# massquantity/dismember

Hardware: AMD Instinct MI355X
Metric: beam-search users/sec + recall@200 vs brute-force, 10M-item tree (higher is better)
Workload: dtype f32; 1 GPU; TDM beam-search serving, synthetic 10000000-item depth-24 binary tree, 128-d emb, beam=200, topk=200, L=10; items=10000000, depth=24, embed=128, beam=200, topk=200, seq_len=10, parallelism=user-sharded x1, replicated table

## Files before the change

dismember_amd/csrc/beam_kernel.hip.inc:

```

#if !defined(DM_PROBE_BUILD) &&                                                                                            \
    (defined(DM_DBG_NO_S) || defined(DM_DBG_NO_GATHER) || defined(DM_DBG_NO_EPI) || defined(DM_DBG_NO_XLANE) ||             \
     defined(DM_SPLIT_NO_MIX) || defined(DMW_DBG_F_NOEPI) || defined(DMW_DBG_F_NOLD) || defined(DMW_DBG_F_NOSM) ||          \
     defined(DMW_DBG_HOTROWS) || defined(DMW_DBG_NOWAIT) || defined(DMW_DBG_NO_GATHER) || defined(DMW_DBG_NO_GVV) ||        \
     defined(DMW_DBG_SM_UPTO) || defined(DM_PHASE_TIMERS) || defined(DM_TILE_TIMERS) || defined(DM_SETUP_TIMERS))
#error "timing knock-outs and in-kernel timers need -DDM_PROBE_BUILD (probe builds only: they change results)"
#endif

typedef float f32x4 __attribute__((ext_vector_type(4)));
typedef _Float16 dm_h8 __attribute__((ext_vector_type(8)));
typedef _Float16 dm_h2 __attribute__((ext_vector_type(2)));

#define DM_BLOCK 512
#define DM_NWAVES 8
#define DM_MAXL 16
#define DM_PIPE_MAXL 32

struct BeamParams {
  const float *emb;
  const f32x4 *wfrag;
  const f32x4 *afrag;
  const f32x4 *bfrag;
  const float *b1, *w2;
  float b2;
  const dm_h8 *wsplit;
  const dm_h8 *emb_split;
  float emb_scale, score_unscale, acc_scale, out_unscale;
  int64_t num_index;
  const uint32_t *exists_bits, *leaf_bits;
  const int32_t *node_id, *id_to_code;
  int64_t n_slots;
  int32_t non_leaf_offset, max_code, max_level;
  int leaf_fast;
  const int32_t *seq;
  int64_t U;
  int L, use_mask, beam, topk, widen;
  const int64_t *consumed_off;
  const int32_t *consumed_ids;
  int mode;
  const int32_t *bf_leaf_codes;
  int64_t bf_n_leaf;
  int bf_slices, bf_chunk;
  int64_t bf_per_slice;
  unsigned long long *bf_out_keys;
  int otm_leaf_level;
  int nteams, cap, pcap;
  int32_t *out_ids;
  float *out_scores;
  int32_t *out_counts;
  int out_stride;
  int32_t *ws_code;
  float *ws_score;
  uint32_t *ws_khi, *ws_klo;
  int ws_cap;
  unsigned long long *next_user;
  int32_t *trace_codes;
  float *trace_scores;
  int32_t *trace_counts;
  int trace_levels;
  unsigned long long *scored_rows;
  unsigned long long *phase_cycles;
  unsigned long long *defer_count;
  int32_t *defer_users;
  const unsigned long long *user_count;
  const int32_t *user_list;
  float sm_scale;
  int static_users;
  int host_direct;
};

__device__ __forceinline__ uint32_t dm_desc_key(float s) {
  uint32_t b = __float_as_uint(s);
  if (s != s) b = 0x7fc00000u;
  uint32_t asc = (b & 0x80000000u) ? ~b : (b | 0x80000000u);
  return ~asc;
}

template <int CTRL>
__device__ __forceinline__ float dm_dpp(float x) {
  return __int_as_float(__builtin_amdgcn_update_dpp(0, __float_as_int(x), CTRL, 0xF, 0xF, true));
}
#ifdef DM_DBG_NO_XLANE
__device__ __forceinline__ float dm_xor16(float x) { return x; }
__device__ __forceinline__ float dm_xor32(float x) { return x; }
#else
__device__ __forceinline__ float dm_xor16(float x) {
  return __int_as_float(__builtin_amdgcn_ds_swizzle(__float_as_int(x), 0x1F | (16 << 10)));
}
__device__ __forceinline__ float dm_xor32(float x) { return __shfl_xor(x, 32); }
#endif
__device__ __forceinline__ float dm_sum16(float x) {
  x += dm_dpp<0xB1>(x);
  x += dm_dpp<0x4E>(x);
  x += dm_dpp<0x141>(x);
  x += dm_dpp<0x140>(x);
  return x;
}
__device__ __forceinline__ float dm_max16(float x) {
  x = fmaxf(x, dm_dpp<0xB1>(x));
  x = fmaxf(x, dm_dpp<0x4E>(x));
  x = fmaxf(x, dm_dpp<0x141>(x));
  x = fmaxf(x, dm_dpp<0x140>(x));
  return x;
}

__device__ __forceinline__ bool dm_bit(const uint32_t *bits, int64_t i) { return (bits[i >> 5] >> (i & 31)) & 1u; }

__device__ __forceinline__ uint32_t dm_xor_lane(uint32_t v, int m) {
  switch (m) {
    case 1: return (uint32_t)__builtin_amdgcn_update_dpp(0, (int)v, 0xB1, 0xF, 0xF, true);
    case 2: return (uint32_t)__builtin_amdgcn_update_dpp(0, (int)v, 0x4E, 0xF, 0xF, true);
    case 4: return (uint32_t)__builtin_amdgcn_ds_swizzle((int)v, 0x1F | (4 << 10));
    case 8: return (uint32_t)__builtin_amdgcn_ds_swizzle((int)v, 0x1F | (8 << 10));
    case 16: return (uint32_t)__builtin_amdgcn_ds_swizzle((int)v, 0x1F | (16 << 10));
    default: return (uint32_t)__shfl_xor((int)v, 32);
  }
}

__device__ __forceinline__ uint32_t dm_xor_lane_valu(uint32_t v, int m, int lane) {
  switch (m) {
    case 1: return (uint32_t)__builtin_amdgcn_update_dpp(0, (int)v, 0xB1, 0xF, 0xF, true);
    case 2: return (uint32_t)__builtin_amdgcn_update_dpp(0, (int)v, 0x4E, 0xF, 0xF, true);
    case 4: {
      const uint32_t a = (uint32_t)__builtin_amdgcn_update_dpp(0, (int)v, 0x124, 0xF, 0xF, true);
      const uint32_t b = (uint32_t)__builtin_amdgcn_update_dpp(0, (int)v, 0x12C, 0xF, 0xF, true);
      return (lane & 4) ? a : b;
    }
    case 8: return (uint32_t)__builtin_amdgcn_update_dpp(0, (int)v, 0x128, 0xF, 0xF, true);
    case 16: { const auto r = __builtin_amdgcn_permlane16_swap(v, v, false, false); return (lane & 16) ? r[0] : r[1]; }
    default: { const auto r = __builtin_amdgcn_permlane32_swap(v, v, false, false); return (lane & 32) ? r[0] : r[1]; }
  }
}

template <int J>
__device__ __forceinline__ void dm_sort_stage(unsigned long long (&key)[4], int lane, int base, int k) {
  if (J == 1) {
#pragma unroll
    for (int e = 0; e < 4; e += 2) {
      const bool asc = ((base + e) & k) == 0;
      const unsigned long long a = key[e], b = key[e + 1];
      const bool sw = (a < b) != asc;
      key[e] = sw ? b : a; key[e + 1] = sw ? a : b;
    }
  } else if (J == 2) {
    const bool asc = (base & k) == 0;
#pragma unroll
    for (int e = 0; e < 2; e++) {
      const unsigned long long a = key[e], b = key[e + 2];
      const bool sw = (a < b) != asc;
      key[e] = sw ? b : a; key[e + 2] = sw ? a : b;
    }
  } else {
    constexpr int M = J / 4;
    const bool keepmin = ((lane & M) == 0) == ((base & k) == 0);
    uint32_t olo[4], ohi[4];
#pragma unroll
    for (int e = 0; e < 4; e++) {
      olo[e] = dm_xor_lane((uint32_t)key[e], M);
      ohi[e] = dm_xor_lane((uint32_t)(key[e] >> 32), M);
    }
#pragma unroll
    for (int e = 0; e < 4; e++) {
      const unsigned long long o = ((unsigned long long)ohi[e] << 32) | olo[e];
      key[e] = ((key[e] < o) == keepmin) ? key[e] : o;
    }
  }
}

struct BeamLds {
  int wfrag, b1, w2, slot0, slot_stride;
  int x_kfrag, x_gfrag;
  int y_keys, y_acode0, y_acode1, y_aval;
  int misc, sync, total;
};
__host__ __device__ inline BeamLds dm_beam_lds(int E, int nteams, int cap, int pcap, int kq, bool split = false, int kt = 1) {
  const int kcols = (kq >= 4 || kt > 1) ? 16 : 12;
  BeamLds l;
  int o = 0;
  l.wfrag = o; o += E * E * 4;
  l.b1 = o; o += E * 4;
// ... 996 lines not shown
```

dismember_amd/csrc/beam_kernel_w.hip.inc:

```

#define DMW_BLOCK 256
#define DMW_NWAVES 4

__device__ __forceinline__ void dmw_mfma_av(f32x4 &acc, const dm_h8 &a, const dm_h8 &b) {
  asm volatile("v_mfma_f32_16x16x32_f16 %0, %1, %2, %0" : "+v"(acc) : "a"(a), "v"(b));
}
__device__ __forceinline__ void dmw_mfma_av0(f32x4 &acc, const dm_h8 &a, const dm_h8 &b) {
  asm volatile("v_mfma_f32_16x16x32_f16 %0, %1, %2, 0" : "+v"(acc) : "a"(a), "v"(b));
}
__device__ __forceinline__ void dmw_mfma_vv(f32x4 &acc, const dm_h8 &a, const dm_h8 &b) {
  asm volatile("v_mfma_f32_16x16x32_f16 %0, %1, %2, %0" : "+v"(acc) : "v"(a), "v"(b));
}
__device__ __forceinline__ void dmw_mfma_vv0(f32x4 &acc, const dm_h8 &a, const dm_h8 &b) {
  asm volatile("v_mfma_f32_16x16x32_f16 %0, %1, %2, 0" : "=&v"(acc) : "v"(a), "v"(b));
}
__device__ __forceinline__ void dmw_mfma_f32(f32x4 &acc, float a, float b) {
  asm volatile("v_mfma_f32_16x16x4_f32 %0, %1, %2, %0" : "+v"(acc) : "v"(a), "v"(b));
}
#define DMW_PIN() __builtin_amdgcn_sched_barrier(0)
template <int OFF>
__device__ __forceinline__ void dmw_gather16(dm_h8 &dst, const dm_h8 *src) {
  asm volatile("global_load_dwordx4 %0, %1, off offset:%2" : "=v"(dst) : "v"(src), "n"(OFF));
}
template <int N>
__device__ __forceinline__ void dmw_vmwait() { asm volatile("s_waitcnt vmcnt(%0)" :: "n"(N)); }

template <typename F, int... I>
__device__ __forceinline__ void dm_static_for_impl(F &&f, std::integer_sequence<int, I...>) { (f(std::integral_constant<int, I>{}), ...); }
template <int N, typename F>
__device__ __forceinline__ void dm_static_for(F &&f) { dm_static_for_impl(f, std::make_integer_sequence<int, N>{}); }
#define DMW_FOR(N, v) dm_static_for<N>([&](auto v##_c) { constexpr int v = decltype(v##_c)::value;
#define DMW_END });

__device__ __forceinline__ void dmw_split_a(const f32x4 &u, const f32x4 &v, float s, unsigned (&h)[4]) {
  asm volatile("v_fma_mixlo_f16 %0, %4, %8, 0 op_sel_hi:[0,0,0]\n\t"
               "v_fma_mixlo_f16 %1, %5, %8, 0 op_sel_hi:[0,0,0]\n\t"
               "v_fma_mixlo_f16 %2, %6, %8, 0 op_sel_hi:[0,0,0]\n\t"
               "v_fma_mixlo_f16 %3, %7, %8, 0 op_sel_hi:[0,0,0]"
               : "=&v"(h[0]), "=&v"(h[1]), "=&v"(h[2]), "=&v"(h[3]) : "v"(u[0]), "v"(u[2]), "v"(v[0]), "v"(v[2]), "v"(s));
}
__device__ __forceinline__ void dmw_split_b(const f32x4 &u, const f32x4 &v, float s, unsigned (&h)[4]) {
  asm volatile("v_fma_mixhi_f16 %0, %4, %8, 0 op_sel_hi:[0,0,0]\n\t"
               "v_fma_mixhi_f16 %1, %5, %8, 0 op_sel_hi:[0,0,0]\n\t"
               "v_fma_mixhi_f16 %2, %6, %8, 0 op_sel_hi:[0,0,0]\n\t"
               "v_fma_mixhi_f16 %3, %7, %8, 0 op_sel_hi:[0,0,0]\n\t"
               "s_nop 0"
               : "+v"(h[0]), "+v"(h[1]), "+v"(h[2]), "+v"(h[3]) : "v"(u[1]), "v"(u[3]), "v"(v[1]), "v"(v[3]), "v"(s));
}
__device__ __forceinline__ void dmw_split_c(const f32x4 &u, const f32x4 &v, float s, const unsigned (&h)[4], unsigned (&l)[4]) {
  asm volatile("v_fma_mixlo_f16 %0, %4, %8, -%9 op_sel:[0,0,0] op_sel_hi:[0,0,1]\n\t"
               "v_fma_mixlo_f16 %1, %5, %8, -%10 op_sel:[0,0,0] op_sel_hi:[0,0,1]\n\t"
               "v_fma_mixlo_f16 %2, %6, %8, -%11 op_sel:[0,0,0] op_sel_hi:[0,0,1]\n\t"
               "v_fma_mixlo_f16 %3, %7, %8, -%12 op_sel:[0,0,0] op_sel_hi:[0,0,1]"
               : "=&v"(l[0]), "=&v"(l[1]), "=&v"(l[2]), "=&v"(l[3])
               : "v"(u[0]), "v"(u[2]), "v"(v[0]), "v"(v[2]), "v"(s), "v"(h[0]), "v"(h[1]), "v"(h[2]), "v"(h[3]));
}
__device__ __forceinline__ void dmw_split_d(const f32x4 &u, const f32x4 &v, float s, const unsigned (&h)[4], unsigned (&l)[4]) {
  asm volatile("v_fma_mixhi_f16 %0, %4, %8, -%9 op_sel:[0,0,1] op_sel_hi:[0,0,1]\n\t"
               "v_fma_mixhi_f16 %1, %5, %8, -%10 op_sel:[0,0,1] op_sel_hi:[0,0,1]\n\t"
               "v_fma_mixhi_f16 %2, %6, %8, -%11 op_sel:[0,0,1] op_sel_hi:[0,0,1]\n\t"
               "v_fma_mixhi_f16 %3, %7, %8, -%12 op_sel:[0,0,1] op_sel_hi:[0,0,1]\n\t"
               "s_nop 0"
               : "+v"(l[0]), "+v"(l[1]), "+v"(l[2]), "+v"(l[3])
               : "v"(u[1]), "v"(u[3]), "v"(v[1]), "v"(v[3]), "v"(s), "v"(h[0]), "v"(h[1]), "v"(h[2]), "v"(h[3]));
}
__device__ __forceinline__ float dmw_split_src(const f32x4 &u, const f32x4 &v, int piece, int i) {
  const int odd = piece & 1;
  return i == 0 ? u[odd] : i == 1 ? u[2 + odd] : i == 2 ? v[odd] : v[2 + odd];
}
__device__ __forceinline__ void dmw_split_1(const f32x4 &u, const f32x4 &v, float s, unsigned (&h)[4], unsigned (&l)[4], int piece, int i) {
  const float x = dmw_split_src(u, v, piece, i);
  if (piece == 0) asm volatile("v_fma_mixlo_f16 %0, %1, %2, 0 op_sel_hi:[0,0,0]" : "=v"(h[i]) : "v"(x), "v"(s));
  else if (piece == 1) asm volatile("v_fma_mixhi_f16 %0, %1, %2, 0 op_sel_hi:[0,0,0]" : "+v"(h[i]) : "v"(x), "v"(s));
  else if (piece == 2) asm volatile("v_fma_mixlo_f16 %0, %1, %2, -%3 op_sel:[0,0,0] op_sel_hi:[0,0,1]" : "=&v"(l[i]) : "v"(x), "v"(s), "v"(h[i]));
  else asm volatile("v_fma_mixhi_f16 %0, %1, %2, -%3 op_sel:[0,0,1] op_sel_hi:[0,0,1]" : "+v"(l[i]) : "v"(x), "v"(s), "v"(h[i]));
}
__device__ __forceinline__ dm_h8 dmw_pack(const unsigned (&x)[4]) {
  typedef unsigned u32x4_ __attribute__((ext_vector_type(4)));
  const u32x4_ v = {x[0], x[1], x[2], x[3]};
  return __builtin_bit_cast(dm_h8, v);
}

template <int MASK>
__device__ __forceinline__ uint32_t dmw_lane_xor(uint32_t v, int lane) {
  if constexpr (MASK == 1) return (uint32_t)__builtin_amdgcn_update_dpp(0, (int)v, 0xB1, 0xF, 0xF, true);
  else if constexpr (MASK == 2) return (uint32_t)__builtin_amdgcn_update_dpp(0, (int)v, 0x4E, 0xF, 0xF, true);
  else if constexpr (MASK == 3) return (uint32_t)__builtin_amdgcn_update_dpp(0, (int)v, 0x1B, 0xF, 0xF, true);
  else if constexpr (MASK == 7) return (uint32_t)__builtin_amdgcn_update_dpp(0, (int)v, 0x141, 0xF, 0xF, true);
  else if constexpr (MASK == 15) return (uint32_t)__builtin_amdgcn_update_dpp(0, (int)v, 0x140, 0xF, 0xF, true);
  else if constexpr (MASK == 4 || MASK == 8 || MASK == 16 || MASK == 31)
    return (uint32_t)__builtin_amdgcn_ds_swizzle((int)v, 0x1F | (MASK << 10));
  else return (uint32_t)__shfl((int)v, lane ^ MASK);
}
#define DMW_KEY_SHIFT 30
#define DMW_KEY_POS(k) ((uint32_t)(k) & 0x3FFFFFFFu)
#define DMW_KEY_PAD 0x7FEFFFFFFFFFFFFFull
__device__ __forceinline__ unsigned long long dmw_make_key(float score, unsigned pos) {
  return ((unsigned long long)dm_desc_key(score) << DMW_KEY_SHIFT) | pos;
}
__device__ __forceinline__ void dmw_cx(unsigned long long &a, unsigned long long &b) {
  unsigned long long lo, hi;
  asm("v_min_f64 %0, %1, %2" : "=v"(lo) : "v"(a), "v"(b));
  asm("v_max_f64 %0, %1, %2" : "=v"(hi) : "v"(a), "v"(b));
  a = lo; b = hi;
}
template <int X>
__device__ __forceinline__ void dmw_sort_inlane(unsigned long long (&key)[8]) {
#pragma unroll
  for (int e = 0; e < 8; e++) if ((e ^ X) > e) dmw_cx(key[e], key[e ^ X]);
}
__device__ __forceinline__ void dmw_sort_role(unsigned long long (&key)[8], unsigned &neg, unsigned want) {
  const unsigned m = neg ^ want;
#pragma unroll
  for (int e = 0; e < 8; e++) key[e] ^= (unsigned long long)m << 32;
  neg = want;
}
template <int LM, bool FLIP>
__device__ __forceinline__ void dmw_sort_xlane(unsigned long long (&key)[8], int lane, unsigned &neg) {
  constexpr int TOP = LM >= 32 ? 32 : LM >= 16 ? 16 : LM >= 8 ? 8 : LM >= 4 ? 4 : LM >= 2 ? 2 : 1;
  dmw_sort_role(key, neg, (lane & TOP) ? 0x80000000u : 0u);
  unsigned long long o[8];
#pragma unroll
  for (int e = 0; e < 8; e++) {
    const uint32_t olo = dmw_lane_xor<LM>((uint32_t)key[e], lane), ohi = dmw_lane_xor<LM>((uint32_t)(key[e] >> 32), lane);
    o[FLIP ? 7 - e : e] = ((unsigned long long)ohi << 32) | olo;
  }
#pragma unroll
  for (int e = 0; e < 8; e++) asm("v_min_f64 %0, %0, -%1" : "+v"(key[e]) : "v"(o[e]));
}
template <int K>
__device__ __forceinline__ void dmw_sort_phase(unsigned long long (&key)[8], int lane, unsigned &neg) {
  if constexpr (K <= 8) dmw_sort_inlane<K - 1>(key);
  else dmw_sort_xlane<K / 8 - 1, true>(key, lane, neg);
  if constexpr (K >= 512) dmw_sort_xlane<16, false>(key, lane, neg);
  if constexpr (K >= 256) dmw_sort_xlane<8, false>(key, lane, neg);
  if constexpr (K >= 128) dmw_sort_xlane<4, false>(key, lane, neg);
  if constexpr (K >= 64) dmw_sort_xlane<2, false>(key, lane, neg);
  if constexpr (K >= 32) dmw_sort_xlane<1, false>(key, lane, neg);
  if constexpr (K >= 16) dmw_sort_role(key, neg, 0u);
  if constexpr (K >= 16) dmw_sort_inlane<4>(key);
  if constexpr (K >= 8) dmw_sort_inlane<2>(key);
  if constexpr (K >= 4) dmw_sort_inlane<1>(key);
}

struct BeamWLds { int b1, w2, slot0, slot_stride, x_kfrag, x_gfrag, y_keys, y_acode0, y_acode1, y_aval, misc, total; };
__host__ __device__ inline BeamWLds dm_beamw_lds(int E, int cap, int pcap, int kq) {
  const int kcols = kq >= 4 ? 16 : 12;
  BeamWLds l;
  int o = 0;
  l.b1 = o; o += E * 4;
  l.w2 = o; o += E * 4;
  l.slot0 = o;
  int s = 0;
  l.x_kfrag = s; s += (E / 16) * 4 * kcols * 16;
  l.x_gfrag = s; s += kq * (E / 16) * 64 * 4 > (E / 16) * 64 * 16 ? kq * (E / 16) * 64 * 4 : (E / 16) * 64 * 16;
  const int ybase = s;
  l.y_keys = s; s += pcap * 8;
  l.y_acode0 = s; s += cap * 4;
  l.y_acode1 = s; s += cap * 4;
  l.y_aval = s; s += cap * 4;
  if (s - ybase < 16 * (E + 4) * 4) s = ybase + 16 * (E + 4) * 4;
  s = (s + 15) & ~15;
  l.misc = s; s += 64 * 4;
  l.slot_stride = s;
  o += s * DMW_NWAVES;
  l.total = (o + 15) & ~15;
  return l;
}

constexpr int dmw_sm_pos(int npos, int k) {
  const int skips = (k > 4 ? 4 : 0) + (k > 5 ? 4 : 0) + (k > 10 ? 4 : 0) + (k > 11 ? 4 : 0);
  return npos >= 64 ? 12 + k + skips : (k * npos) / 18;
}
constexpr int dmw_sp_slot(int nslot, int gps, int s, int piece) { const int b = 3 * gps * (s + 1) + piece; return b < nslot ? b : nslot - 1; }
constexpr int dmw_ep_slot(int nb, int j) { const int last = 3 * (j / nb) - 1, first = 3 * (j / nb - 1); return first + ((j % nb) * (last - first + 1)) / nb; }

template <int E, int KQ>
__global__ __launch_bounds__(DMW_BLOCK, 1) void dm_beam_w_kernel(BeamParams p) {
  constexpr int NJ = E / 16, NT = E / 16, NS = E / 32;
  constexpr int KCOLS = KQ >= 4 ? 16 : 12;
  constexpr int NB = NT < 4 ? NT : 4;
  constexpr int NGRP = NS * (NT / NB);
  extern __shared__ __attribute__((aligned(16))) char smem[];
  const BeamWLds lo = dm_beamw_lds(E, p.cap, p.pcap, KQ);
  const int tid = threadIdx.x, lane = tid & 63, wave = tid >> 6;
  const int CAP = p.cap, L = p.L;
  float *B1 = (float *)(smem + lo.b1), *W2 = (float *)(smem + lo.w2);
  char *slotp = smem + lo.slot0 + wave * lo.slot_stride;
  unsigned long long *keys = (unsigned long long *)(slotp + lo.y_keys);
  float *A_val = (float *)(slotp + lo.y_aval);
  int *misc = (int *)(slotp + lo.misc);
  const dm_h8 *Kh = (const dm_h8 *)(slotp + lo.x_kfrag);
  const float *Gf = (const float *)(slotp + lo.x_gfrag);

  dm_h8 wreg[2 * NS * NT];
#pragma unroll
  for (int i = 0; i < 2 * NS * NT; i++) {
    const dm_h8 t = p.wsplit[i * 64 + lane];
    asm volatile("" : "=a"(wreg[i]) : "0"(t));
  }
  for (int i = tid; i < E; i += DMW_BLOCK) { B1[i] = p.b1[i]; W2[i] = p.w2[i] * p.out_unscale; }
  __syncthreads();
  const float scale2 = (float)(1.4426950408889634 * (double)p.sm_scale) * p.score_unscale;
  unsigned long long my_rows = 0;
#ifdef DM_PHASE_TIMERS
  unsigned long long tph[8] = {0, 0, 0, 0, 0, 0, 0, 0};
  unsigned long long tlast = clock64();
#define WMARK(k) do { unsigned long long tn_ = clock64(); tph[k] += tn_ - tlast; tlast = tn_; } while (0)
#else
#define WMARK(k) do {} while (0)
#endif
#ifdef DM_SETUP_TIMERS
  unsigned long long tsu[8] = {0, 0, 0, 0, 0, 0, 0, 0};
  unsigned long long ts_last = 0;
#define SMARK(k) do { unsigned long long tn_ = clock64(); if (k >= 0) tsu[k < 0 ? 0 : k] += tn_ - ts_last; ts_last = tn_; } while (0)
#else
#define SMARK(k) do {} while (0)
#endif
#ifdef DM_TILE_TIMERS
  unsigned long long ttile[8] = {0, 0, 0, 0, 0, 0, 0, 0};
  unsigned long long tt_last = 0;
#define TMARK(k) do { unsigned long long tn_ = clock64(); ttile[k] += tn_ - tt_last; tt_last = tn_; } while (0)
#else
#define TMARK(k) do {} while (0)
#endif

  auto wsync = [&]() {
    __builtin_amdgcn_fence(__ATOMIC_RELEASE, "wavefront");
    __builtin_amdgcn_wave_barrier();
    __builtin_amdgcn_fence(__ATOMIC_ACQUIRE, "wavefront");
  };
  auto scan4 = [&](unsigned bits4, int &total) -> int {
    const unsigned long long below = (lane == 0) ? 0ull : (~0ull >> (64 - lane));
    int before = 0, wtot = 0;
#pragma unroll
    for (int j = 0; j < 4; j++) {
      const unsigned long long m = __ballot((bits4 >> j) & 1u);
      before += __popcll(m & below);
      wtot += __popcll(m);
    }
    total = wtot;
    return before;
  };
  auto scan8 = [&](unsigned bits8, int &total) -> int {
    const unsigned long long below = (lane == 0) ? 0ull : (~0ull >> (64 - lane));
    int before = 0, wtot = 0;
#pragma unroll
    for (int j = 0; j < 8; j++) {
      const unsigned long long m = __ballot((bits8 >> j) & 1u);
      before += __popcll(m & below);
      wtot += __popcll(m);
    }
    total = wtot;
    return before;
  };
  auto reg_sort8 = [&](unsigned long long (&key)[8], int Pn) {
    int ln = lane;
    asm volatile("" : "+v"(ln));
    unsigned neg = 0u;
    dmw_sort_phase<2>(key, ln, neg);
    dmw_sort_phase<4>(key, ln, neg);
    dmw_sort_phase<8>(key, ln, neg);
    if (Pn >= 16) dmw_sort_phase<16>(key, ln, neg);
    if (Pn >= 32) dmw_sort_phase<32>(key, ln, neg);
    if (Pn >= 64) dmw_sort_phase<64>(key, ln, neg);
    if (Pn >= 128) dmw_sort_phase<128>(key, ln, neg);
    if (Pn >= 256) dmw_sort_phase<256>(key, ln, neg);
    if (Pn >= 512) dmw_sort_phase<512>(key, ln, neg);
  };
  auto lds_sort = [&](int P) {
    for (int k = 2; k <= P; k <<= 1)
      for (int j = k >> 1; j > 0; j >>= 1) {
        wsync();
        for (int c = lane; c < (P >> 1); c += 64) {
          const int i = ((c & ~(j - 1)) << 1) | (c & (j - 1)), l2 = i + j;
          const unsigned long long a = keys[i], b = keys[l2];
          const bool asc = (i & k) == 0;
          const unsigned long long mn = a < b ? a : b, mx = a < b ? b : a;
          keys[i] = asc ? mn : mx; keys[l2] = asc ? mx : mn;
        }
      }
    wsync();
  };
  auto store_keys8 = [&](const unsigned long long (&key)[8], int ln) {
    const int i0 = 8 * ln;
    if (i0 < p.pcap) {
      *(ulonglong2 *)(keys + i0) = make_ulonglong2(key[0], key[1]);
      *(ulonglong2 *)(keys + i0 + 2) = make_ulonglong2(key[2], key[3]);
      *(ulonglong2 *)(keys + i0 + 4) = make_ulonglong2(key[4], key[5]);
      *(ulonglong2 *)(keys + i0 + 6) = make_ulonglong2(key[6], key[7]);
    }
  };

  const int64_t wsb = ((int64_t)blockIdx.x * DMW_NWAVES + wave) * p.ws_cap;

  for (;;) {
    long long user;
    {
      unsigned long long u = 0;
      if (lane == 0) u = atomicAdd(p.next_user, 1ull);
      u = ((unsigned long long)__builtin_amdgcn_readfirstlane((int)(u >> 32)) << 32) | (unsigned)__builtin_amdgcn_readfirstlane((int)u);
      user = u < (unsigned long long)p.U ? (long long)u : -1;
    }
    if (user < 0) break;
    WMARK(6);

    SMARK(-1);
    if (lane == 0) {
      int beam = p.beam;
      if (p.widen && p.consumed_off) {
        const int nc = (int)(p.consumed_off[user + 1] - p.consumed_off[user]);
        const int w = (nc + p.topk) / 2;
        beam = w > beam ? w : beam;
        if (2 * beam > CAP) beam = CAP / 2;
      }
      const int level = 31 - __clz(beam);
      const int start = (1 << level) - 1;
      int n_iter = p.mode == 0 ? p.max_level - level + 1 : p.otm_leaf_level - level;
      if (n_iter < 0) n_iter = 0;
      if (n_iter > 34) n_iter = 34;
      misc[M_BEAM] = beam; misc[M_START] = start; misc[M_NITER] = n_iter; misc[M_LVOFF] = 0; misc[M_KEPT] = 0;
      misc[M_GMAX] = 0; misc[M_GSP] = DM_G32;
    }
    {
      int32_t code = -1;
      if (lane < L) {
        const int32_t id = p.seq[user * L + lane];
        if (p.mode == 1) code = id;
        else if (id == 0) code = -1;
        else if (id < p.non_leaf_offset && id >= 0 && p.id_to_code[id] >= 0) code = p.id_to_code[id];
        else {
          const int32_t t = (int32_t)((uint32_t)id - (uint32_t)p.non_leaf_offset);
          code = (t > p.max_code) ? -1 : t;
        }
        if (code < -1 || code >= p.num_index) code = -1;
        misc[M_SEQ + lane] = code;
      }
      const unsigned pm = (unsigned)__ballot(lane < L && code == -1);
      if (lane == 0) misc[M_PADMASK] = p.use_mask ? pm : 0u;
    }
    wsync();
    SMARK(0);
    {
      const int r = lane & 15, g = lane >> 4;
      const int32_t kcode = (r < L) ? misc[M_SEQ + r] : -1;
      f32x4 ka[NJ];
      if (kcode >= 0) {
        const f32x4 *src = (const f32x4 *)(p.emb + (int64_t)kcode * E) + g;
#pragma unroll
        for (int jc = 0; jc < NJ; jc++) ka[jc] = src[4 * jc];
      } else {
#pragma unroll
        for (int jc = 0; jc < NJ; jc++) ka[jc] = (f32x4){0.f, 0.f, 0.f, 0.f};
      }
      if (r < KCOLS) {
        dm_h8 *Khw = (dm_h8 *)(slotp + lo.x_kfrag);
#pragma unroll
        for (int s = 0; s < NS; s++) {
          dm_h8 hi, lw;
          dm_split8(ka[2 * s], ka[2 * s + 1], p.emb_scale, hi, lw);
          Khw[(s * 4 + g) * KCOLS + r] = hi;
          Khw[((NS + s) * 4 + g) * KCOLS + r] = lw;
        }
      }
      SMARK(1);
      float *T1s = (float *)(slotp + lo.y_keys);
      auto gemm16 = [&](const f32x4 *frag, const f32x4 (&a)[NJ], auto &&emit) {
        f32x4 bq[3][NJ];
        unsigned lo16 = 16u * (unsigned)lane;
        asm volatile("" : "+v"(lo16));
        const char *fb = (const char *)frag;
        auto fetch = [&](auto nt_c) {
          constexpr int nt = decltype(nt_c)::value;
#pragma unroll
          for (int jc = 0; jc < NJ; jc++) bq[nt % 3][jc] = *(const f32x4 *)(fb + (size_t)((jc * NT + nt) * 1024) + lo16);
        };
        fetch(std::integral_constant<int, 0>{});
        if constexpr (NT > 1) fetch(std::integral_constant<int, 1>{});
        DMW_FOR(NT, nt)
          if constexpr (nt + 2 < NT) fetch(std::integral_constant<int, nt + 2>{});
          f32x4 acc = {0.f, 0.f, 0.f, 0.f};
          asm volatile("s_nop 1" : "+v"(acc));
#pragma unroll
          for (int jc = 0; jc < NJ; jc++)
#pragma unroll
            for (int t = 0; t < 4; t++) dmw_mfma_f32(acc, a[jc][t], bq[nt % 3][jc][t]);
          asm volatile("s_nop 7\n\ts_nop 7" : "+v"(acc));
          emit(nt, acc);
        DMW_END
      };
      gemm16(p.afrag, ka, [&](int nt, const f32x4 &acc) {
#pragma unroll
        for (int rr = 0; rr < 4; rr++) T1s[(4 * g + rr) * (E + 4) + 16 * nt + r] = acc[rr];
      });
      wsync();
      SMARK(2);
      f32x4 ta[NJ];
#pragma unroll
      for (int jc = 0; jc < NJ; jc++) ta[jc] = *(const f32x4 *)(T1s + r * (E + 4) + 16 * jc + 4 * g);
      float *Gfw = (float *)(slotp + lo.x_gfrag);
      float gm = 0.0f;
      gemm16(p.bfrag, ta, [&](int nt, const f32x4 &acc) {
        if (g < KQ) {
          const float bb = B1[16 * nt + r];
#pragma unroll
          for (int rr = 0; rr < 4; rr++) {
            const float gv = (4 * g + rr < L) ? acc[rr] + bb : 0.0f;
            Gfw[(g * NT + nt) * 64 + rr * 16 + r] = gv;
            gm = __builtin_fmaxf(gm, __builtin_fabsf(gv));
          }
        }
      });
      SMARK(3);
      unsigned gbits = __float_as_uint(gm);
      gbits = gbits < 0x7f800000u ? gbits : 0x7f800000u;
      for (int o = 32; o > 0; o >>= 1) { const unsigned t_ = (unsigned)__shfl_xor((int)gbits, o); gbits = t_ > gbits ? t_ : gbits; }
      wsync();
      const int S = (int)((__float_as_uint(p.acc_scale) >> 23) & 0xff) - 127;
      int sp = DM_G32;
      if (gbits < 0x7f800000u) {
        const int e = gbits ? (int)(gbits >> 23) - 126 : -126;
        sp = S - (14 - e);
        if (sp < -10) sp = -10;
        if (sp > 15) sp = DM_G32;
      }
      constexpr int NENT = NT * 64;
      constexpr int NQ = (NENT + 63) / 64;
      if (sp != DM_G32) {
        const float gs = __uint_as_float((unsigned)(S - sp + 127) << 23);
        float gv[NQ][4];
#pragma unroll
        for (int q = 0; q < NQ; q++) {
          const int idx = lane + 64 * q;
          const int nt_ = (idx >> 6) % NT, m_ = idx & 15, g_ = (idx >> 4) & 3;
#pragma unroll
          for (int i = 0; i < 4; i++) {
            const int pos = g_ + 4 * i;
            gv[q][i] = ((pos >> 2) < KQ) ? Gfw[((pos >> 2) * NT + nt_) * 64 + (pos & 3) * 16 + m_] * gs : 0.0f;
          }
        }
        wsync();
        typedef float f32x2_ __attribute__((ext_vector_type(2)));
#pragma unroll
        for (int q = 0; q < NQ; q++) {
          const int idx = lane + 64 * q;
          const dm_h2 h01 = __builtin_convertvector((f32x2_){gv[q][0], gv[q][1]}, dm_h2);
          const dm_h2 h23 = __builtin_convertvector((f32x2_){gv[q][2], gv[q][3]}, dm_h2);
          const dm_h2 l01 = __builtin_convertvector((f32x2_){gv[q][0] - (float)h01[0], gv[q][1] - (float)h01[1]}, dm_h2);
          const dm_h2 l23 = __builtin_convertvector((f32x2_){gv[q][2] - (float)h23[0], gv[q][3] - (float)h23[1]}, dm_h2);
          dm_h8 o;
          o[0] = h01[0]; o[1] = h01[1]; o[2] = h23[0]; o[3] = h23[1]; o[4] = l01[0]; o[5] = l01[1]; o[6] = l23[0]; o[7] = l23[1];
          ((dm_h8 *)Gfw)[idx] = o;
        }
      } else {
        for (int i = lane; i < KQ * NT * 64; i += 64) Gfw[i] *= p.acc_scale;
      }
      if (lane == 0) misc[M_GSP] = sp;
    }
    wsync();
    SMARK(4);
    if (__builtin_amdgcn_readfirstlane(misc[M_GSP]) == DM_G32) {
      if (lane == 0) { const unsigned long long q = atomicAdd(p.defer_count, 1ull); p.defer_users[q] = (int32_t)user; }
      continue;
    }
    int n_cand;
    {
      const int start = misc[M_START];
      const int n_iter0 = misc[M_NITER];
      int32_t *A0 = (int32_t *)(slotp + lo.y_acode0);
      int base = 0;
      for (int r0 = 0; r0 < CAP / 2; r0 += 256) {
        unsigned bits = 0;
#pragma unroll
        for (int j = 0; j < 4; j++) {
          const int i = r0 + 4 * lane + j;
          const int64_t code = (int64_t)start + i;
          bool ok = n_iter0 > 0 && i <= start;
          if (ok && p.mode == 0) ok = code < p.n_slots && dm_bit(p.exists_bits, code);
          bits |= ok ? (1u << j) : 0u;
        }
        int total;
        const int before = scan4(bits, total);
#pragma unroll
        for (int j = 0; j < 4; j++)
          if ((bits >> j) & 1u) {
            const int q = base + before + __popc(bits & ((1u << j) - 1));
            A0[q] = start + r0 + 4 * lane + j; A_val[q] = 0.0f;
          }
        base += total;
      }
      n_cand = base;
    }
    wsync();

    const int n_iter = misc[M_NITER];
    const int beam = misc[M_BEAM];
    const unsigned padmask = (unsigned)misc[M_PADMASK];
    const int gsp = __builtin_amdgcn_readfirstlane(misc[M_GSP]);
    const float pscale = gsp != DM_G32 ? __uint_as_float((unsigned)(gsp + 127) << 23) : 1.0f;
    int cur = 0;
    int leaf_tot = 0;
    SMARK(5);
    WMARK(0);

    for (int it = 0; it < n_iter; it++) {
      int32_t *Acur = (int32_t *)(slotp + (cur ? lo.y_acode1 : lo.y_acode0));
      int32_t *Anext = (int32_t *)(slotp + (cur ? lo.y_acode0 : lo.y_acode1));
      const int n = n_cand;
      const bool first = (it == 0);
      int m_nl = n;
      int leaf_base = leaf_tot;
      int nchild = 0;
      int ln = lane;
      asm volatile("" : "+v"(ln));
      if (p.mode == 0) {
        if (p.leaf_fast) {
          if (it == n_iter - 1) {
            for (int i = ln; i < n; i += 64) {
              const int q = leaf_base + i;
              if (q < p.ws_cap) { p.ws_code[wsb + q] = Acur[i]; p.ws_score[wsb + q] = A_val[i]; }
            }
            leaf_base += n; m_nl = 0;
          }
        } else {
          int nl = 0;
          for (int r0 = 0; r0 < n; r0 += 256) {
            unsigned lbits = 0, nbits = 0;
            int32_t cc[4]; float vv[4];
#pragma unroll
            for (int j = 0; j < 4; j++) {
              const int i = r0 + 4 * ln + j;
              const bool valid = i < n;
              cc[j] = valid ? Acur[i] : 0; vv[j] = valid ? A_val[i] : 0.0f;
              const bool isleaf = valid && dm_bit(p.leaf_bits, cc[j]);
              lbits |= isleaf ? (1u << j) : 0u;
              nbits |= (valid && !isleaf) ? (1u << j) : 0u;
            }
            int tl, tn;
            const int bl = scan4(lbits, tl);
            const int bn = scan4(nbits, tn);
            wsync();
#pragma unroll
            for (int j = 0; j < 4; j++) {
              if ((nbits >> j) & 1u) { const int q = nl + bn + __popc(nbits & ((1u << j) - 1)); Acur[q] = cc[j]; A_val[q] = vv[j]; }
              if ((lbits >> j) & 1u) {
                const int q = leaf_base + bl + __popc(lbits & ((1u << j) - 1));
                if (q < p.ws_cap) { p.ws_code[wsb + q] = cc[j]; p.ws_score[wsb + q] = vv[j]; }
              }
            }
            nl += tn; leaf_base += tl;
            wsync();
          }
          m_nl = nl;
        }
        leaf_tot = leaf_base;
        if (lane == 0) misc[M_LVOFF + it + 1] = leaf_base;
      }
      const bool do_sort = (p.mode == 0) ? (m_nl > beam) : !first;
      const int nb = do_sort ? (m_nl < beam ? m_nl : beam) : m_nl;
      if (do_sort) {
        int P = 2;
        while (P < m_nl) P <<= 1;
        if (P <= 512) {
          unsigned long long key[8];
          const int rd = 8 * ln + 8 <= CAP ? 8 * ln : 0;
// ... 546 lines not shown
```

dismember_amd/csrc/dm_hip.hip:

```cpp
#include "../../include/dismember_hip.h"

#include <hip/hip_runtime.h>

#include <algorithm>
#include <array>
#include <atomic>
#include <mutex>
#include <thread>
#include <utility>
#include <cerrno>
#include <chrono>
#include <cfloat>
#include <cmath>
#include <cstdio>
#include <cstdlib>
#include <cstring>
#include <string>
#include <vector>

#ifdef DM_DEV_LIGHT
#define DM_IF_ALL_E(...)
#else
#define DM_IF_ALL_E(...) __VA_ARGS__
#endif
// ... 1169 lines not shown
  const int n = NS * NT * 64 * 8;
  for (int t = blockIdx.x * blockDim.x + threadIdx.x; t < n; t += gridDim.x * blockDim.x) {
    const int i = t & 7, lane = (t >> 3) & 63, nt = (t >> 9) % NT, s = (t >> 9) / NT;
    const int jc = 2 * s + (i >> 2);
    const float x = wfrag[(((size_t)jc * NT + nt) * 64 + lane) * 4 + (i & 3)] * scale;
    const _Float16 hi = (_Float16)x;
    const _Float16 lo = (_Float16)(x - (float)hi);
    planes[t] = hi;
    planes[(size_t)n + t] = lo;
  }
}

__global__ void dm_build_emb_split_kernel(const float *emb, int64_t num_index, int E, float scale, _Float16 *out) {
  const int64_t n8 = num_index * (int64_t)(E / 8);
  for (int64_t t = (int64_t)blockIdx.x * blockDim.x + threadIdx.x; t < n8; t += (int64_t)gridDim.x * blockDim.x) {
    const int64_t row = t / (E / 8);
    const int sg = (int)(t % (E / 8)), s_ = sg >> 2, g = sg & 3;
    const float *src = emb + row * E + 32 * s_ + 4 * g;
    _Float16 *dst = out + row * (int64_t)(2 * E) + (int64_t)sg * 16;
#pragma unroll
    for (int i = 0; i < 8; i++) {
      const float x = src[16 * (i >> 2) + (i & 3)] * scale;
      const _Float16 hi = (_Float16)x;
      dst[i] = hi;
      dst[8 + i] = (_Float16)(x - (float)hi);
    }
  }
}

__global__ void dm_maxabs_rows_kernel(const float *emb, const int32_t *rows, int64_t n_rows, int E, unsigned *out) {
  unsigned m = 0;
  const int64_t n = n_rows * E;
  for (int64_t t = (int64_t)blockIdx.x * blockDim.x + threadIdx.x; t < n; t += (int64_t)gridDim.x * blockDim.x) {
    const unsigned b = __float_as_uint(emb[(int64_t)rows[t / E] * E + (t % E)]) & 0x7fffffffu;
    m = b > m ? b : m;
  }
  for (int o = 32; o > 0; o >>= 1) { const unsigned t = (unsigned)__shfl_xor((int)m, o); m = t > m ? t : m; }
  if ((threadIdx.x & 63) == 0 && m) atomicMax(out, m);
}
__global__ void dm_build_emb_split_rows_kernel(const float *emb, const int32_t *rows, int64_t n_rows, int E, float scale, _Float16 *out) {
  const int64_t n8 = n_rows * (int64_t)(E / 8);
  for (int64_t t = (int64_t)blockIdx.x * blockDim.x + threadIdx.x; t < n8; t += (int64_t)gridDim.x * blockDim.x) {
    const int64_t row = rows[t / (E / 8)];
    const int sg = (int)(t % (E / 8)), s_ = sg >> 2, g = sg & 3;
    const float *src = emb + row * E + 32 * s_ + 4 * g;
    _Float16 *dst = out + row * (int64_t)(2 * E) + (int64_t)sg * 16;
#pragma unroll
    for (int i = 0; i < 8; i++) {
      const float x = src[16 * (i >> 2) + (i & 3)] * scale;
      const _Float16 hi = (_Float16)x;
      dst[i] = hi;
      dst[8 + i] = (_Float16)(x - (float)hi);
    }
  }
}

static int split_shift(unsigned maxbits) {
  if (maxbits == 0 || maxbits >= 0x7f800000u) return 0;
  float m;
  memcpy(&m, &maxbits, 4);
  int e;
  frexpf(m, &e);
  int sh = 14 - e;
  if (sh > 40) sh = 40;
  if (sh < -40) sh = -40;
  return sh;
}

static int ensure_split_scales(dm_ctx *h) {
  std::lock_guard<std::recursive_mutex> lk_(h->mu);
  if (!h->split_dirty && h->d_wsplit) return DM_OK;
  model_changed(h);
  const int E = h->embed;
  if (E % 32 != 0) return fail(h, DM_ERR_UNSUPPORTED, "the split-fp16 scorer needs an embedding size that is a multiple of 32");
  if (!h->d_wsplit) ALLOC(h, h->d_wsplit, (size_t)E * E * 4);
  if (!h->d_maxabs) ALLOC(h, h->d_maxabs, 8);
  bool patch = h->train_ready && h->sh_e_valid && !h->table_dense_change && h->d_active_list && h->dtype == DM_F32;
  unsigned mb[2];
  for (;;) {
    HIPCHK(h, hipMemsetAsync(h->d_maxabs, 0, 8, h->stream));
    if (patch) {
      if (h->active_rows_host)
        hipLaunchKernelGGL(dm_maxabs_rows_kernel, dim3(1024), dim3(256), 0, h->stream, h->d_emb32, h->d_active_list, (int64_t)h->active_rows_host, E, h->d_maxabs);
    } else
      hipLaunchKernelGGL(dm_maxabs_kernel, dim3(4096), dim3(256), 0, h->stream, h->d_emb32, h->num_index * (int64_t)E, h->d_maxabs);
    hipLaunchKernelGGL(dm_maxabs_kernel, dim3(16), dim3(256), 0, h->stream, (const float *)h->d_wfrag, (int64_t)E * E, h->d_maxabs + 1);
    HIPCHK(h, hipGetLastError());
    HIPCHK(h, hipMemcpyAsync(mb, h->d_maxabs, 8, hipMemcpyDeviceToHost, h->stream));
    HIPCHK(h, hipStreamSynchronize(h->stream));
    if (patch && mb[0] != 0 && split_shift(mb[0]) < h->sh_e) { patch = false; continue; }
    break;
  }
  if (!patch) {
    h->sh_e = split_shift(mb[0]);
    h->sh_e_valid = true; h->table_dense_change = false; h->emb_split_need_full = true;
  }
  h->emb_split_patch = patch;
  h->sh_w = split_shift(mb[1]);
  hipLaunchKernelGGL(dm_build_wsplit_kernel, dim3(64), dim3(256), 0, h->stream, (const float *)h->d_wfrag, E, ldexpf(1.0f, h->sh_w),
                     (_Float16 *)h->d_wsplit);
  HIPCHK(h, hipGetLastError());
  h->split_dirty = false;
  h->emb_split_dirty = true;
  h->rows_split_dirty = true;
  return DM_OK;
}

static int ensure_split(dm_ctx *h) {
  std::lock_guard<std::recursive_mutex> lk_(h->mu);
  int rc = ensure_split_scales(h);
  if (rc != DM_OK) return rc;
  if (!h->emb_split_dirty && h->d_emb_split) return DM_OK;
  model_changed(h);
  const int E = h->embed;
  const size_t bytes = (size_t)h->num_index * E * 4;
  if (h->emb_split_bytes != bytes) {
    dm_free_ptr(h->d_emb_split); h->d_emb_split = nullptr; h->emb_split_bytes = 0;
    ALLOC(h, h->d_emb_split, bytes);
    h->emb_split_bytes = bytes;
    h->emb_split_need_full = true;
  }
  if (h->emb_split_need_full || !h->emb_split_patch) {
    hipLaunchKernelGGL(dm_build_emb_split_kernel, dim3(8192), dim3(256), 0, h->stream, h->d_emb32, h->num_index, E, ldexpf(1.0f, h->sh_e),
                       (_Float16 *)h->d_emb_split);
    h->emb_split_need_full = false;
  } else if (h->active_rows_host) {
    hipLaunchKernelGGL(dm_build_emb_split_rows_kernel, dim3(1024), dim3(256), 0, h->stream, h->d_emb32, h->d_active_list, (int64_t)h->active_rows_host,
                       E, ldexpf(1.0f, h->sh_e), (_Float16 *)h->d_emb_split);
  }
  HIPCHK(h, hipGetLastError());
  h->emb_split_dirty = false;
  return DM_OK;
}

static int ensure_f32_mirror(dm_ctx *h);
static int launch_beam(dm_ctx *h, BeamParams &p, const SearchPlan &pl) {
  if (p.host_direct && p.mode != 0) return fail(h, DM_ERR_STATE, "launch_beam: the host-mapped single-request path is a mode-0 (TDM) path");
  {
    const bool was = h->f32_mirror_dirty;
    int rc_ = ensure_f32_mirror(h);
    if (rc_ != DM_OK) return rc_;
    if (was) p.b2 = h->b2;
  }
  if (h->scorer_mode == DM_SCORER_SPLIT_F16 && h->embed % 32 != 0)
    return fail(h, DM_ERR_UNSUPPORTED, "the split-fp16 scorer needs an embedding size of 32, 64 or 128");
  if (h->call_split && p.mode != 2) {
    int rc = ensure_split(h);
    if (rc != DM_OK) return rc;
    p.wsplit = (const dm_h8 *)h->d_wsplit;
    p.emb_split = (const dm_h8 *)h->d_emb_split;
    p.emb_scale = ldexpf(1.0f, h->sh_e); p.score_unscale = ldexpf(1.0f, -2 * h->sh_e);
    p.acc_scale = ldexpf(1.0f, h->sh_e + h->sh_w); p.out_unscale = ldexpf(1.0f, -(h->sh_e + h->sh_w));
    if (pl.wkernel) {
      const size_t need = 16 + (size_t)p.U * 4;
      if (h->defer_bytes < need) {
        dm_free_ptr(h->d_defer); h->d_defer = nullptr; h->defer_bytes = 0;
        ALLOC(h, h->d_defer, need + need / 4);
        h->defer_bytes = need + need / 4;
      }
      HIPCHK(h, hipMemsetAsync(h->d_defer, 0, 16, h->stream));
      p.defer_count = (unsigned long long *)h->d_defer;
      p.defer_users = (int32_t *)((char *)h->d_defer + 16);
      int rc = DM_OK;
      switch (h->embed) {
        DM_IF_ALL_E(case 32: rc = launch_beam_w_E<32>(h, p, pl); break;)
        DM_IF_ALL_E(case 64: rc = launch_beam_w_E<64>(h, p, pl); break;)
        default: rc = launch_beam_w_E<128>(h, p, pl); break;
      }
      if (rc != DM_OK) return rc;
      SearchPlan pl2;
      {
        const int kq = (p.L + 3) / 4;
        int nteams = 0;
        for (int cand = 4; cand >= 1; cand >>= 1) {
          BeamLds l = dm_beam_lds(h->embed, cand, pl.cap, pl.pcap, kq, true);
          if (l.total <= 160 * 1024) { nteams = cand; pl2.lds = l.total; break; }
        }
        if (!nteams) return fail(h, DM_ERR_UNSUPPORTED, "beam too large for the LDS frontier");
        pl2 = pl; pl2.nteams = nteams; pl2.wkernel = false;
        BeamLds l = dm_beam_lds(h->embed, nteams, pl.cap, pl.pcap, kq, true);
        pl2.lds = l.total;
        if (pl2.grid * pl2.nteams > pl.grid * pl.nteams) pl2.grid = pl.grid * pl.nteams / pl2.nteams;
        if (pl2.grid < 1) pl2.grid = 1;
      }
      BeamParams p2 = p;
      p2.nteams = pl2.nteams;
      p2.user_count = (const unsigned long long *)h->d_defer;
      p2.user_list = (const int32_t *)((char *)h->d_defer + 16);
      p2.next_user = (unsigned long long *)((char *)h->d_defer + 8);
      p2.defer_count = nullptr; p2.defer_users = nullptr;
      h->ev_next_kind = 1;
      switch (h->embed) {
        DM_IF_ALL_E(case 32: rc = launch_beam_E<32, true>(h, p2, pl2); break;)
        DM_IF_ALL_E(case 64: rc = launch_beam_E<64, true>(h, p2, pl2); break;)
        default: rc = launch_beam_E<128, true>(h, p2, pl2); break;
      }
      h->ev_next_kind = 0;
      return rc;
    }
    switch (h->embed) {
      DM_IF_ALL_E(case 32: return launch_beam_E<32, true>(h, p, pl);)
      DM_IF_ALL_E(case 64: return launch_beam_E<64, true>(h, p, pl);)
      case 128: return launch_beam_E<128, true>(h, p, pl);
    }
    return fail(h, DM_ERR_UNSUPPORTED, "the split-fp16 scorer needs an embedding size of 32, 64 or 128");
  }
  switch (h->embed) {
    DM_IF_ALL_E(case 16: return launch_beam_E<16, false>(h, p, pl);)
    DM_IF_ALL_E(case 32: return launch_beam_E<32, false>(h, p, pl);)
    DM_IF_ALL_E(case 64: return launch_beam_E<64, false>(h, p, pl);)
    case 128: return launch_beam_E<128, false>(h, p, pl);
  }
  return fail(h, DM_ERR_UNSUPPORTED, "unsupported embed size");
}

int dm_set_scorer_mode(dm_handle_t h, int mode) {
  if (!h) return DM_ERR_INVALID;
  if (mode != DM_SCORER_F32 && mode != DM_SCORER_SPLIT_F16 && mode != DM_SCORER_AUTO && mode != DM_SCORER_F64) return fail(h, DM_ERR_INVALID, "dm_set_scorer_mode: unknown mode");
  if (mode == DM_SCORER_F64 && h->w_loaded && h->dtype != DM_F64)
    return fail(h, DM_ERR_UNSUPPORTED, "dm_set_scorer_mode: the fp64 scorer needs f64 weights");
  if (mode == DM_SCORER_SPLIT_F16 && h->w_loaded && h->embed % 32 != 0)
    return fail(h, DM_ERR_UNSUPPORTED, "dm_set_scorer_mode: the split-fp16 scorer needs an embedding size of 32, 64 or 128");
  h->scorer_mode = mode;
  if (h->parent) h->seen_epoch = 0;
  return DM_OK;
}

int dm_get_scorer_mode(dm_handle_t h, int *mode, int *effective, int *shift_emb, int *shift_w) {
  if (!h || !mode) return DM_ERR_INVALID;
  *mode = h->scorer_mode;
  if (effective) *effective = (h->w_loaded && use_f64_beam(h)) ? DM_SCORER_F64 : (h->w_loaded && use_split(h)) ? DM_SCORER_SPLIT_F16 : DM_SCORER_F32;
  if (shift_emb) *shift_emb = h->sh_e;
  if (shift_w) *shift_w = h->sh_w;
  return DM_OK;
}

static void fill_common(dm_ctx *h, BeamParams &p) {
  memset(&p, 0, sizeof p);
  p.emb = h->d_emb32; p.wfrag = h->d_wfrag; p.afrag = h->d_afrag; p.bfrag = h->d_bfrag; p.b1 = h->d_b1; p.w2 = h->d_w2;
  p.b2 = h->b2; p.num_index = h->num_index;
  p.exists_bits = h->d_exists; p.leaf_bits = h->d_leaf; p.node_id = h->d_node_id; p.id_to_code = h->d_id_to_code;
  p.n_slots = h->n_slots; p.non_leaf_offset = h->non_leaf_offset; p.max_code = h->max_code; p.max_level = h->max_level;
  p.scored_rows = h->d_rows;
  p.sm_scale = sm_scale32(h);
  p.phase_cycles = h->d_phase;
  p.next_user = h->d_rows + 1;
}

static int tdm_pipeline_dev(dm_ctx *h, const int32_t *d_seq, int64_t U, int L, const dm_tdm_search_opts *o, int max_beam,
                            const int64_t *d_coff, const int32_t *d_cids, int32_t *d_ids, float *d_scores, int32_t *d_counts,
                            int trace_levels, int cap, int32_t *d_tc, float *d_ts, int32_t *d_tn);

static int tdm_search_dev(dm_ctx *h, const int32_t *d_seq, int64_t U, int L, const dm_tdm_search_opts *o, int max_beam,
                          const int64_t *d_coff, const int32_t *d_cids, int32_t *d_ids, float *d_scores, int32_t *d_counts,
                          int trace_levels, int32_t *d_tc, float *d_ts, int32_t *d_tn, bool *direct = nullptr) {
  if (!h->tree_loaded || !h->ids_loaded || !h->w_loaded) return fail(h, DM_ERR_STATE, "tdm beam search: tree, id maps and weights must be loaded first");
  if (U < 0 || L <= 0 || L > DM_PIPE_MAXL || !o || o->beam <= 0 || o->topk <= 0) return fail(h, DM_ERR_INVALID, "tdm beam search: bad arguments (L must be 1..32)");
  if (U == 0) return DM_OK;
  if (h->n_slots > h->num_index) return fail(h, DM_ERR_INDEX, "tdm beam search: tree codes exceed the embedding table (embeddingLookup would fail)");
  if (h->max_code >= h->num_index) return fail(h, DM_ERR_INDEX, "tdm beam search: id map codes exceed the embedding table");
  if (long_history_pipeline(h, max_beam, L)) {
    if (direct) { *direct = false; return DM_OK; }
    HIPCHK(h, hipMemsetAsync(d_ids, 0xFF, (size_t)U * o->topk * 4, h->stream));
    HIPCHK(h, hipMemsetAsync(d_scores, 0, (size_t)U * o->topk * 4, h->stream));
    HIPCHK(h, hipMemsetAsync(d_counts, 0, (size_t)U * 4, h->stream));
    const int cap_ = ((2 * max_beam + 15) / 16) * 16 < 32 ? 32 : ((2 * max_beam + 15) / 16) * 16;
    return tdm_pipeline_dev(h, d_seq, U, L, o, max_beam, d_coff, d_cids, d_ids, d_scores, d_counts, trace_levels, cap_, d_tc, d_ts, d_tn);
  }
  int start, level;
  level_start_int(o->beam, &start, &level);
  int n_levels = h->max_level - level + 1;
  if (n_levels < 0) n_levels = 0;
  SearchPlan pl;
  int rc = plan_search(h, max_beam, U, L, n_levels, true, &pl);
  if (rc != DM_OK) return rc;
  const size_t per = (size_t)pl.grid * pl.nteams * pl.ws_cap;
  rc = ensure_ws(h, per * 16);
  if (rc != DM_OK) return rc;
  BeamParams p;
  fill_common(h, p);
  p.seq = d_seq; p.U = U; p.L = L; p.use_mask = o->use_mask; p.beam = o->beam; p.topk = o->topk;
  p.widen = (o->widen_consumed && d_coff) ? 1 : 0;
  p.consumed_off = d_coff; p.consumed_ids = d_cids; p.mode = 0; p.nteams = pl.nteams; p.cap = pl.cap; p.pcap = pl.pcap; p.leaf_fast = h->leaves_at_max_only ? 1 : 0;
  p.out_ids = d_ids; p.out_scores = d_scores; p.out_counts = d_counts; p.out_stride = o->topk;
  p.ws_code = (int32_t *)h->d_ws; p.ws_score = (float *)h->d_ws + per; p.ws_khi = (uint32_t *)h->d_ws + 2 * per;
  p.ws_klo = (uint32_t *)h->d_ws + 3 * per; p.ws_cap = pl.ws_cap;
  p.trace_codes = d_tc; p.trace_scores = d_ts; p.trace_counts = d_tn; p.trace_levels = trace_levels;
  if (direct) {
    *direct = *direct && !pl.wkernel && U <= (int64_t)pl.grid * pl.nteams && !d_coff && !d_tn;
    if (!*direct) return DM_OK;
    {
      p.host_direct = 1;
      p.scored_rows = h->d_rows + 3;
      h->ev_skip = true;
      const int rc_ = launch_beam(h, p, pl);
      h->ev_skip = false;
      return rc_;
    }
  }
  if (h->rows_keep) HIPCHK(h, hipMemsetAsync(h->d_rows + 1, 0, 8, h->stream));
  else HIPCHK(h, hipMemsetAsync(h->d_rows, 0, 16, h->stream));
  HIPCHK(h, hipMemsetAsync(d_ids, 0xFF, (size_t)U * o->topk * 4, h->stream));
  HIPCHK(h, hipMemsetAsync(d_scores, 0, (size_t)U * o->topk * 4, h->stream));
  HIPCHK(h, hipMemsetAsync(d_counts, 0, (size_t)U * 4, h->stream));
  return launch_beam(h, p, pl);
}
// ... 555 lines not shown
```

Baseline: 1.724 million users/s.

## Fuse two-stage f32 setup GEMMs into one split-fp16 MFMA GEMM with prefetch ring

Replaces the per-user setup that ran two chained f32 16x16x4 MFMA GEMMs (key*A into an LDS staging tile, then a wave sync, then *B) with a single GEMM against a precombined matrix stored as split hi/lo fp16. It uses 16x16x32 f16 MFMAs with the hi*hi + hi*lo + lo*hi split, and software-prefetches the matrix fragments through a register ring of configurable depth. The intent is to cut the MFMA count, the LDS round-trip and sync, and the padding of the staging area in LDS. The cost is extra register pressure from the ring and possible precision loss, since the lo*lo term is dropped. It also depends on ensure_rows_split providing the combined matrix at the assumed offset.

```diff
diff --git a/dismember_amd/csrc/beam_kernel.hip.inc b/dismember_amd/csrc/beam_kernel.hip.inc
--- a/dismember_amd/csrc/beam_kernel.hip.inc
+++ b/dismember_amd/csrc/beam_kernel.hip.inc
@@ -26,6 +26,8 @@
   const dm_h8 *wsplit;
   const dm_h8 *emb_split;
   float emb_scale, score_unscale, acc_scale, out_unscale;
+  const dm_h8 *msplit;
+  float m_unscale;
   int64_t num_index;
   const uint32_t *exists_bits, *leaf_bits;
   const int32_t *node_id, *id_to_code;
diff --git a/dismember_amd/csrc/beam_kernel_w.hip.inc b/dismember_amd/csrc/beam_kernel_w.hip.inc
--- a/dismember_amd/csrc/beam_kernel_w.hip.inc
+++ b/dismember_amd/csrc/beam_kernel_w.hip.inc
@@ -1,5 +1,8 @@
 
 #define DMW_BLOCK 256
+#ifndef DMW_SETUP_RING
+#define DMW_SETUP_RING 4
+#endif
 #define DMW_NWAVES 4
 
 __device__ __forceinline__ void dmw_mfma_av(f32x4 &acc, const dm_h8 &a, const dm_h8 &b) {
@@ -17,6 +20,8 @@
 __device__ __forceinline__ void dmw_mfma_f32(f32x4 &acc, float a, float b) {
   asm volatile("v_mfma_f32_16x16x4_f32 %0, %1, %2, %0" : "+v"(acc) : "v"(a), "v"(b));
 }
+__device__ __forceinline__ void dmw_mfma_drain(f32x4 &acc) { asm volatile("s_nop 7\n\ts_nop 7" : "+v"(acc)); }
+__device__ __forceinline__ void dmw_opaque(f32x4 &acc) { asm volatile("" : "+v"(acc)); }
 #define DMW_PIN() __builtin_amdgcn_sched_barrier(0)
 template <int OFF>
 __device__ __forceinline__ void dmw_gather16(dm_h8 &dst, const dm_h8 *src) {
@@ -154,12 +159,10 @@
   int s = 0;
   l.x_kfrag = s; s += (E / 16) * 4 * kcols * 16;
   l.x_gfrag = s; s += kq * (E / 16) * 64 * 4 > (E / 16) * 64 * 16 ? kq * (E / 16) * 64 * 4 : (E / 16) * 64 * 16;
-  const int ybase = s;
   l.y_keys = s; s += pcap * 8;
   l.y_acode0 = s; s += cap * 4;
   l.y_acode1 = s; s += cap * 4;
   l.y_aval = s; s += cap * 4;
-  if (s - ybase < 16 * (E + 4) * 4) s = ybase + 16 * (E + 4) * 4;
   s = (s + 15) & ~15;
   l.misc = s; s += 64 * 4;
   l.slot_stride = s;
@@ -343,6 +346,21 @@
     SMARK(0);
     {
       const int r = lane & 15, g = lane >> 4;
+      constexpr int NBS = NT < 4 ? NT : 4, NGS = NT / NBS, NSTEP = NGS * NS;
+      constexpr int RING = DMW_SETUP_RING < NSTEP ? DMW_SETUP_RING : NSTEP;
+      unsigned lo16 = 16u * (unsigned)lane;
+      asm volatile("" : "+v"(lo16));
+      const char *mbase = (const char *)p.msplit;
+      dm_h8 mb[RING][NBS][2];
+      auto fetch_m = [&](auto q_c) {
+        constexpr int q = decltype(q_c)::value, s_ = q % NS, nt0 = (q / NS) * NBS;
+#pragma unroll
+        for (int i = 0; i < NBS; i++)
+#pragma unroll
+          for (int h = 0; h < 2; h++)
+            mb[q % RING][i][h] = *(const dm_h8 *)(mbase + (size_t)(((h * NS + s_) * NT + nt0 + i) * 1024) + lo16);
+      };
+      DMW_FOR(RING, q) fetch_m(q_c); DMW_END
       const int32_t kcode = (r < L) ? misc[M_SEQ + r] : -1;
       f32x4 ka[NJ];
       if (kcode >= 0) {
@@ -353,64 +371,44 @@
 #pragma unroll
         for (int jc = 0; jc < NJ; jc++) ka[jc] = (f32x4){0.f, 0.f, 0.f, 0.f};
       }
+      dm_h8 kh[NS], kl[NS];
+#pragma unroll
+      for (int s = 0; s < NS; s++) dm_split8(ka[2 * s], ka[2 * s + 1], p.emb_scale, kh[s], kl[s]);
       if (r < KCOLS) {
         dm_h8 *Khw = (dm_h8 *)(slotp + lo.x_kfrag);
 #pragma unroll
         for (int s = 0; s < NS; s++) {
-          dm_h8 hi, lw;
-          dm_split8(ka[2 * s], ka[2 * s + 1], p.emb_scale, hi, lw);
-          Khw[(s * 4 + g) * KCOLS + r] = hi;
-          Khw[((NS + s) * 4 + g) * KCOLS + r] = lw;
+          Khw[(s * 4 + g) * KCOLS + r] = kh[s];
+          Khw[((NS + s) * 4 + g) * KCOLS + r] = kl[s];
         }
       }
       SMARK(1);
-      float *T1s = (float *)(slotp + lo.y_keys);
-      auto gemm16 = [&](const f32x4 *frag, const f32x4 (&a)[NJ], auto &&emit) {
-        f32x4 bq[3][NJ];
-        unsigned lo16 = 16u * (unsigned)lane;
-        asm volatile("" : "+v"(lo16));
-        const char *fb = (const char *)frag;
-        auto fetch = [&](auto nt_c) {
-          constexpr int nt = decltype(nt_c)::value;
-#pragma unroll
-          for (int jc = 0; jc < NJ; jc++) bq[nt % 3][jc] = *(const f32x4 *)(fb + (size_t)((jc * NT + nt) * 1024) + lo16);
-        };
-        fetch(std::integral_constant<int, 0>{});
-        if constexpr (NT > 1) fetch(std::integral_constant<int, 1>{});
-        DMW_FOR(NT, nt)
-          if constexpr (nt + 2 < NT) fetch(std::integral_constant<int, nt + 2>{});
-          f32x4 acc = {0.f, 0.f, 0.f, 0.f};
-          asm volatile("s_nop 1" : "+v"(acc));
-#pragma unroll
-          for (int jc = 0; jc < NJ; jc++)
-#pragma unroll
-            for (int t = 0; t < 4; t++) dmw_mfma_f32(acc, a[jc][t], bq[nt % 3][jc][t]);
-          asm volatile("s_nop 7\n\ts_nop 7" : "+v"(acc));
-          emit(nt, acc);
-        DMW_END
-      };
-      gemm16(p.afrag, ka, [&](int nt, const f32x4 &acc) {
-#pragma unroll
-        for (int rr = 0; rr < 4; rr++) T1s[(4 * g + rr) * (E + 4) + 16 * nt + r] = acc[rr];
-      });
-      wsync();
-      SMARK(2);
-      f32x4 ta[NJ];
-#pragma unroll
-      for (int jc = 0; jc < NJ; jc++) ta[jc] = *(const f32x4 *)(T1s + r * (E + 4) + 16 * jc + 4 * g);
       float *Gfw = (float *)(slotp + lo.x_gfrag);
       float gm = 0.0f;
-      gemm16(p.bfrag, ta, [&](int nt, const f32x4 &acc) {
+      DMW_FOR(NGS, gg)
+        f32x4 acc[NBS];
+        DMW_FOR(NS, s)
+          constexpr int q = gg * NS + s, sl = q % RING;
+          DMW_FOR(NBS, i) if constexpr (s == 0) dmw_mfma_vv0(acc[i], kh[s], mb[sl][i][0]); else dmw_mfma_vv(acc[i], kh[s], mb[sl][i][0]); DMW_END
+          DMW_FOR(NBS, i) dmw_mfma_vv(acc[i], kh[s], mb[sl][i][1]); DMW_END
+          DMW_FOR(NBS, i) dmw_mfma_vv(acc[i], kl[s], mb[sl][i][0]); DMW_END
+          if constexpr (q + RING < NSTEP) fetch_m(std::integral_constant<int, q + RING>{});
+        DMW_END
+        dmw_mfma_drain(acc[0]);
+        DMW_FOR(NBS, i) dmw_opaque(acc[i]); DMW_END
         if (g < KQ) {
-          const float bb = B1[16 * nt + r];
-#pragma unroll
-          for (int rr = 0; rr < 4; rr++) {
-            const float gv = (4 * g + rr < L) ? acc[rr] + bb : 0.0f;
-            Gfw[(g * NT + nt) * 64 + rr * 16 + r] = gv;
-            gm = __builtin_fmaxf(gm, __builtin_fabsf(gv));
-          }
-        }
-      });
+          DMW_FOR(NBS, i)
+            constexpr int nt = gg * NBS + i;
+            const float bb = B1[16 * nt + r];
+#pragma unroll
+            for (int rr = 0; rr < 4; rr++) {
+              const float gv = (4 * g + rr < L) ? acc[i][rr] * p.m_unscale + bb : 0.0f;
+              Gfw[(g * NT + nt) * 64 + rr * 16 + r] = gv;
+              gm = __builtin_fmaxf(gm, __builtin_fabsf(gv));
+            }
+          DMW_END
+        }
+      DMW_END
       SMARK(3);
       unsigned gbits = __float_as_uint(gm);
       gbits = gbits < 0x7f800000u ? gbits : 0x7f800000u;
diff --git a/dismember_amd/csrc/dm_hip.hip b/dismember_amd/csrc/dm_hip.hip
--- a/dismember_amd/csrc/dm_hip.hip
+++ b/dismember_amd/csrc/dm_hip.hip
@@ -1345,6 +1345,10 @@
     p.emb_scale = ldexpf(1.0f, h->sh_e); p.score_unscale = ldexpf(1.0f, -2 * h->sh_e);
     p.acc_scale = ldexpf(1.0f, h->sh_e + h->sh_w); p.out_unscale = ldexpf(1.0f, -(h->sh_e + h->sh_w));
     if (pl.wkernel) {
+      const int rc_m = ensure_rows_split(h);
+      if (rc_m != DM_OK) return rc_m;
+      p.msplit = (const dm_h8 *)h->d_rows_split + (size_t)2 * (h->embed / 32) * (h->embed / 16) * 64;
+      p.m_unscale = ldexpf(1.0f, -(h->sh_e + h->sh_r));
       const size_t need = 16 + (size_t)p.U * 4;
       if (h->defer_bytes < need) {
         dm_free_ptr(h->d_defer); h->d_defer = nullptr; h->defer_bytes = 0;
```

New measurement: 1.740 million users/s, median of 6. No clear change (+1.0%).
